# eth-cscs/conflux

Measured on NVIDIA H100. Metric: LU GFLOP/s (FP64, (2/3)N^3), higher is better.
Workload: dtype f64

## Files before the change

conflux_b200/csrc/dbg.cu:

```cuda
#include <algorithm>
#include <climits>
#include <limits>
#include <vector>

#include "../../include/conflux_b200.h"
#include "common.cuh"
#include "kernels.h"
#include "lu_state.h"

using namespace cflx;

namespace {
struct DevBuf {
    void* p = nullptr;
    ~DevBuf() { cudaFree(p); }
    int alloc(size_t bytes) {
        CFLX_CUDA(cudaMalloc(&p, bytes + 4096));
        return CFLX_OK;
    }
    template <class T>
    T* as() { return (T*)p; }
};
int check_device() {
    int n = 0;
// ... 366 lines not shown
    CFLX_TRY(dXc.alloc(sizeof(double) * (size_t)Nl * nrhs));
    CFLX_TRY(dXr.alloc(sizeof(double) * (size_t)Ml * nrhs));
    CFLX_TRY(dP.alloc(sizeof(double) * o_n));
    CFLX_TRY(dQ.alloc(sizeof(double) * o_n));
    CFLX_CUDA(cudaMemcpy(dA.p, A, sizeof(double) * a_n, cudaMemcpyHostToDevice));
    if (Xc) CFLX_CUDA(cudaMemcpy(dXc.p, Xc, sizeof(double) * (size_t)Nl * nrhs, cudaMemcpyHostToDevice));
    if (Xr) CFLX_CUDA(cudaMemcpy(dXr.p, Xr, sizeof(double) * (size_t)Ml * nrhs, cudaMemcpyHostToDevice));
    const Layout L{0, v, Kappa, Ml, Nl, Px, Py, pi, pj};
    auto run = [&]() {
        return launch_residual(m, dA.as<double>(), L, dXc.as<double>(), dXr.as<double>(), nrhs, nrhs, dP.as<double>(),
                               dQ.as<double>(), nrhs, 0);
    };
    cudaEvent_t e0, e1;
    CFLX_CUDA(cudaEventCreate(&e0));
    CFLX_CUDA(cudaEventCreate(&e1));
    if (reps < 1) reps = 1;
    CFLX_TRY(run());
    CFLX_CUDA(cudaEventRecord(e0));
    for (int r = 0; r < reps; ++r) CFLX_TRY(run());
    CFLX_CUDA(cudaEventRecord(e1));
    CFLX_CUDA(cudaEventSynchronize(e1));
    float ms = 0;
    CFLX_CUDA(cudaEventElapsedTime(&ms, e0, e1));
    if (ms_out) *ms_out = ms / reps;
    cudaEventDestroy(e0);
    cudaEventDestroy(e1);
    CFLX_CUDA(cudaMemset(dP.p, 0, sizeof(double) * o_n));
    CFLX_CUDA(cudaMemset(dQ.p, 0, sizeof(double) * o_n));
    CFLX_TRY(run());
    if (P_out) CFLX_CUDA(cudaMemcpy(P_out, dP.p, sizeof(double) * (size_t)rows * nrhs, cudaMemcpyDeviceToHost));
    if (Q_out) CFLX_CUDA(cudaMemcpy(Q_out, dQ.p, sizeof(double) * (size_t)rows * nrhs, cudaMemcpyDeviceToHost));
    CFLX_CUDA(cudaDeviceSynchronize());
    return CFLX_OK;
}

int cflx_dbg_panel(int n, int v, const double* panel, int* perm_out, double* A00_out, double* LU_out, int reps,
                   double* ms_out) {
    CFLX_TRY(check_device());
    if (n < 0 || v <= 0) return CFLX_ERR_ARG;
    const int64_t ld = std::max<int64_t>(2, round_up(n, 2));
    std::vector<double> WT((size_t)v * ld, 0.0);
    for (int r = 0; r < n; ++r)
        for (int c = 0; c < v; ++c) WT[(size_t)c * ld + r] = panel[(size_t)r * v + c];
    DevBuf dW, dW0, dA00, dA00T, dperm;
    CFLX_TRY(dW.alloc(sizeof(double) * v * ld));
    CFLX_TRY(dW0.alloc(sizeof(double) * v * ld));
    CFLX_TRY(dA00.alloc(sizeof(double) * v * v));
    CFLX_TRY(dA00T.alloc(sizeof(double) * v * v));
    CFLX_TRY(dperm.alloc(sizeof(int) * 2 * v));
    CFLX_CUDA(cudaMemcpy(dW0.p, WT.data(), sizeof(double) * v * ld, cudaMemcpyHostToDevice));
    CFLX_CUDA(cudaMemset(dA00.p, 0, sizeof(double) * v * v));
    PanelWorkspace ws{};
    CFLX_TRY(panel_workspace_create(&ws));
    cudaEvent_t e0, e1;
    CFLX_CUDA(cudaEventCreate(&e0));
    CFLX_CUDA(cudaEventCreate(&e1));
    if (reps < 1) reps = 1;
    float total = 0;
    int nb = 0, rc = CFLX_OK;
    for (int r = 0; r < reps + 1 && rc == CFLX_OK; ++r) {
        cudaMemcpyAsync(dW.p, dW0.p, sizeof(double) * v * ld, cudaMemcpyDeviceToDevice, 0);
        cudaEventRecord(e0);
        rc = launch_panel_getrf_a00(dW.as<double>(), ld, n, v, dperm.as<int>(), dA00.as<double>(), &nb, &ws, 0);
        cudaEventRecord(e1);
        if (cudaEventSynchronize(e1) != cudaSuccess) rc = CFLX_ERR_CUDA;
        float ms = 0;
        cudaEventElapsedTime(&ms, e0, e1);
        if (r > 0) total += ms;
    }
    cudaEventDestroy(e0);
    cudaEventDestroy(e1);
    if (rc == CFLX_OK && n >= v)
        rc = launch_gather_a00(dW.as<double>(), ld, dperm.as<int>(), v, nb, dA00.as<double>(), dA00T.as<double>(), 0);
    panel_workspace_destroy(&ws);
    if (rc != CFLX_OK) {
        if (rc == CFLX_ERR_CUDA) set_last_error("panel kernel failed: %s", cudaGetErrorString(cudaGetLastError()));
        return rc;
    }
    if (ms_out) *ms_out = total / reps;
    if (perm_out) CFLX_CUDA(cudaMemcpy(perm_out, dperm.p, sizeof(int) * v, cudaMemcpyDeviceToHost));
    if (A00_out) CFLX_CUDA(cudaMemcpy(A00_out, dA00.p, sizeof(double) * v * v, cudaMemcpyDeviceToHost));
    if (LU_out) {
        CFLX_CUDA(cudaMemcpy(WT.data(), dW.p, sizeof(double) * v * ld, cudaMemcpyDeviceToHost));
        for (int r = 0; r < n; ++r)
            for (int c = 0; c < v; ++c) LU_out[(size_t)r * v + c] = WT[(size_t)c * ld + r];
    }
    CFLX_CUDA(cudaDeviceSynchronize());
    return CFLX_OK;
}

int cflx_dbg_trsm(int n, int v, int nb, int64_t ld, const double* A00, const double* B, double* X_out, const double* R,
                  double* Y_out) {
    CFLX_TRY(check_device());
    if (n <= 0 || v <= 0 || v % 4 != 0) return CFLX_ERR_ARG;
    if (nb == 0)
        for (int c : {128, 64, 32, 16, 8, 4})
            if (!nb && v % c == 0) nb = c;
    if (nb != 4 && nb != 8 && nb != 16 && nb != 32 && nb != 64 && nb != 128) return CFLX_ERR_UNSUPPORTED;
    if (v % nb != 0) return CFLX_ERR_ARG;
    if (ld == 0) ld = round_up(n, 2);
    if ((ld & 1) || ld < round_up(n, 2)) return CFLX_ERR_ARG;
    const double nan = std::numeric_limits<double>::quiet_NaN();
    std::vector<double> A00T((size_t)v * v), BT((size_t)v * ld, nan), RT((size_t)v * ld, nan);
    for (int i = 0; i < v; ++i)
        for (int j = 0; j < v; ++j) A00T[(size_t)j * v + i] = A00[(size_t)i * v + j];
    DevBuf dA, dAT, dUinv, dLinvT, dP, dL, dR, dU;
// ... 191 lines not shown
```

conflux_b200/csrc/lu.cu:

```cuda
#include <algorithm>
#include <cmath>
#include <cstdarg>
#include <cstdlib>
#include <cstring>
#include <random>
#include <string>
#include <vector>

#include <nvtx3/nvToolsExt.h>

#include "lu_state.h"

namespace cflx {
static thread_local char g_err[1024] = "";
void set_last_error(const char* fmt, ...) {
    va_list ap;
    va_start(ap, fmt);
    vsnprintf(g_err, sizeof(g_err), fmt, ap);
    va_end(ap);
}
}

using namespace cflx;

// ... 811 lines not shown
    lu->a0_is_next = false;
    lu->next_host = nullptr;
    lu->eq.in.equed = 'N';
    return CFLX_OK;
}

int cflx_lu_queue_next_local(cflx_lu* lu, const double* host_next) {
    if (!lu || !host_next) return CFLX_ERR_ARG;
    if (!lu->have_input) {
        set_last_error("cflx_lu_queue_next_local needs a current input (cflx_lu_set_local) first");
        return CFLX_ERR_STATE;
    }
    CFLX_CUDA(cudaSetDevice(lu->comm->device));
    if (!lu->copy) {
        CFLX_CUDA(cudaStreamCreateWithFlags(&lu->copy, cudaStreamNonBlocking));
        CFLX_CUDA(cudaEventCreateWithFlags(&lu->ev_a0_read, cudaEventDisableTiming));
        CFLX_CUDA(cudaEventCreateWithFlags(&lu->ev_upload, cudaEventDisableTiming));
    }
    lu->next_host = host_next;
    return CFLX_OK;
}

int cflx_lu_factor(cflx_lu* lu, double* ms_out) {
    if (!lu) return CFLX_ERR_ARG;
    if (!lu->have_input) {
        set_last_error("cflx_lu_factor before cflx_lu_set_local");
        return CFLX_ERR_STATE;
    }
    cflx_comm* c = lu->comm;
    cudaStream_t s = c->stream;
    CFLX_CUDA(cudaSetDevice(c->device));
    const size_t loc = (size_t)lu->Ml * lu->Nl;
    {
        PhaseTimer t(lu, RG_init, s);
        if (lu->a0_is_next) CFLX_CUDA(cudaStreamWaitEvent(s, lu->ev_upload, 0));
        CFLX_CUDA(cudaMemcpyAsync(lu->A11, lu->A0, loc * sizeof(double), cudaMemcpyDeviceToDevice, s));
    }
    lu->a0_is_next = false;
    lu->sv.ready = false;
    CFLX_TRY(equil_pass_on(&lu->eq, lu->M, lu->next_host != nullptr, s));
    if (lu->next_host) {
        CFLX_CUDA(cudaEventRecord(lu->ev_a0_read, s));
        CFLX_CUDA(cudaStreamWaitEvent(lu->copy, lu->ev_a0_read, 0));
        CFLX_CUDA(cudaMemcpyAsync(lu->A0, lu->next_host, loc * sizeof(double), cudaMemcpyHostToDevice, lu->copy));
        CFLX_CUDA(cudaEventRecord(lu->ev_upload, lu->copy));
        lu->next_host = nullptr;
        lu->a0_is_next = true;
    }
    CFLX_TRY(launch_iota_gri(lu->gri, lu->igri, lu->Ml, lu->v, lu->Px, lu->pi, s));
    for (double& x : lu->phase_ms) x = 0;
    for (int sd = 0; sd < 2; ++sd)
        for (int r = 0; r < RG_COUNT; ++r) lu->region_ms[sd][r] = 0, lu->region_cnt[sd][r] = 0;
    lu->tl_recs.clear();
    CFLX_TRY(grid_barrier(c));
    cudaEvent_t e0, e1;
    CFLX_CUDA(cudaEventCreate(&e0));
    CFLX_CUDA(cudaEventCreate(&e1));
    CFLX_CUDA(cudaEventRecord(e0, s));
    int fnpr = 0;
    lu->gemm_flops = 0;
    lu->gemm_ms = 0;
    if (lu->time_gemm && (int)lu->ev.size() < 4 * lu->Nt) {
        for (auto& e : lu->ev) cudaEventDestroy(e);
        lu->ev.assign(4 * lu->Nt, nullptr);
        for (auto& e : lu->ev) CFLX_CUDA(cudaEventCreate(&e));
    }
    lu->ev_used.assign(2 * lu->Nt, 0);
    {
        cudaStream_t side = (lu->prof_mode == 1) ? nullptr : lu->side;
        if (side) {
            CFLX_CUDA(cudaEventRecord(lu->ev_fork, s));
            CFLX_CUDA(cudaStreamWaitEvent(side, lu->ev_fork, 0));
        }
        int rc0 = panel_phase(lu, 0, 0, side ? side : s);
        if (rc0 != CFLX_OK) return rc0;
        if (side) {
            CFLX_CUDA(cudaEventRecord(lu->ev_join, side));
            CFLX_CUDA(cudaStreamWaitEvent(s, lu->ev_join, 0));
        }
    }
    for (int k = 0; k < lu->Nt; ++k) {
        int rc = finish_step(lu, k, fnpr);
        if (rc != CFLX_OK) {
            cudaEventDestroy(e0);
            cudaEventDestroy(e1);
            return rc;
        }
    }
    CFLX_CUDA(cudaEventRecord(e1, s));
    CFLX_CUDA(cudaEventSynchronize(e1));
    float ms = 0;
    CFLX_CUDA(cudaEventElapsedTime(&ms, e0, e1));
    cudaEventDestroy(e0);
    cudaEventDestroy(e1);
    CFLX_CUDA(cudaGetLastError());
    if (ms_out) *ms_out = ms;
    if (lu->prof_mode == 2) {
        if (lu->side) cudaStreamSynchronize(lu->side);
        for (const auto& r : lu->tl_recs) {
            float g = 0;
            if (cudaEventElapsedTime(&g, lu->tl_pool[r.ev], lu->tl_pool[r.ev + 1]) == cudaSuccess) {
                lu->region_ms[r.side][r.region] += g;
                lu->region_cnt[r.side][r.region]++;
                lu->phase_ms[region_phase(r.region)] += g;
            } else {
                cudaGetLastError();
            }
        }
    }
    if (lu->time_gemm) {
        for (int i = 0; i < 2 * lu->Nt; ++i) {
            if (!lu->ev_used[i]) continue;
            float g = 0;
            if (cudaEventElapsedTime(&g, lu->ev[2 * i], lu->ev[2 * i + 1]) == cudaSuccess) lu->gemm_ms += g;
            else cudaGetLastError();
        }
    }
    if (lu->a0_is_next) CFLX_CUDA(cudaStreamSynchronize(lu->copy));
    lu->factored = true;
    return CFLX_OK;
}

int cflx_lu_get_permutation(cflx_lu* lu, int* perm_out) {
    if (!lu || !perm_out) return CFLX_ERR_ARG;
    CFLX_TRY(lu_check(lu, "permutation", false));
    CFLX_CUDA(cudaSetDevice(lu->comm->device));
    CFLX_CUDA(cudaMemcpyAsync(lu->h_hist.data(), lu->hist, sizeof(int) * lu->M, cudaMemcpyDeviceToHost, lu->comm->stream));
    CFLX_CUDA(cudaStreamSynchronize(lu->comm->stream));
    std::memcpy(perm_out, lu->h_hist.data(), sizeof(int) * lu->M);
    return CFLX_OK;
}

int cflx_lu_get_factors(cflx_lu* lu, double* C_host, int* perm_out) {
    if (!lu) return CFLX_ERR_ARG;
    CFLX_TRY(lu_check(lu, "factors", false));
    cflx_comm* c = lu->comm;
    cudaStream_t s = c->stream;
    CFLX_CUDA(cudaSetDevice(c->device));
    std::vector<int> hist(lu->M);
    CFLX_TRY(cflx_lu_get_permutation(lu, hist.data()));
    if (perm_out) std::memcpy(perm_out, hist.data(), sizeof(int) * lu->M);
    if (lu->pk != 0) return CFLX_OK;
    const size_t loc = (size_t)lu->Ml * lu->Nl;
    if (!lu->Cbuf) CFLX_TRY(dmalloc(&lu->Cbuf, loc));
    CFLX_TRY(redistribute_pivoted_rows(lu, hist, true, lu->A11, lu->Cbuf));
    if (C_host) CFLX_CUDA(cudaMemcpyAsync(C_host, lu->Cbuf, loc * sizeof(double), cudaMemcpyDeviceToHost, s));
    CFLX_CUDA(cudaStreamSynchronize(s));
    return CFLX_OK;
}

int cflx_lu_validate(cflx_lu* lu, double* frob_abs_out, double* frob_rel_out) {
    if (!lu) return CFLX_ERR_ARG;
    CFLX_TRY(lu_check(lu, "residual", true));
    CFLX_CUDA(cudaSetDevice(lu->comm->device));
    std::vector<int> hist(lu->M);
    CFLX_TRY(cflx_lu_get_permutation(lu, hist.data()));
    return lu_residual_grid(lu, hist, frob_abs_out, frob_rel_out);
// ... 98 lines not shown
    CFLX_TRY(lu_rcond(lu, t, &rcond, nullptr));
    *rcond_out = rcond;
    const double *r = rowequ ? eq.r : nullptr, *c = colequ ? eq.c : nullptr;
    const RefineOp op = lu_refine_op(lu, t);
    if (!t) CFLX_TRY(svx_tail(&lu->eq, &lu->sv.rf, op, nrhs, B, ldb, X, ldx, ferr_out, berr_out, r, c, eq.colcnd));
    else CFLX_TRY(svx_tail(&lu->eq, &lu->sv.rf, op, nrhs, B, ldb, X, ldx, ferr_out, berr_out, c, r, eq.rowcnd));
    if (rcond < std::ldexp(1.0, -53)) *info_out = lu->M + 1;
    return CFLX_OK;
}

int cflx_host_alloc(size_t bytes, void** out) {
    if (!out) return CFLX_ERR_ARG;
    int n = 0;
    cflx_device_count(&n);
    if (n == 0) {
        set_last_error("no CUDA device visible: conflux_b200 has no CPU fallback");
        return CFLX_ERR_NO_DEVICE;
    }
    CFLX_CUDA(cudaHostAlloc(out, bytes, cudaHostAllocPortable));
    return CFLX_OK;
}
int cflx_host_free(void* p) {
    if (p) CFLX_CUDA(cudaFreeHost(p));
    return CFLX_OK;
}

int cflx_lu_uses_ozaki(const cflx_lu* lu) { return lu && lu->use_ozaki ? 1 : 0; }
int cflx_lu_launch_count(cflx_lu* lu, int64_t* count_out, int reset) {
    if (!lu || !count_out) return CFLX_ERR_ARG;
    *count_out = lu->launches;
    if (reset) lu->launches = 0;
    return CFLX_OK;
}
int cflx_lu_set_profiling(cflx_lu* lu, int mode) {
    if (!lu || mode < 0 || mode > 2) return CFLX_ERR_ARG;
    lu->prof_mode = mode;
    return CFLX_OK;
}
int cflx_lu_timeline(cflx_lu* lu, char* buf, int buf_len) {
    if (!lu) return CFLX_ERR_ARG;
    std::string o = "{";
    for (int sd = 0; sd < 2; ++sd) {
        o += sd ? ", \"side\": {" : "\"main\": {";
        bool first = true;
        for (int r = 0; r < RG_COUNT; ++r) {
            if (!lu->region_cnt[sd][r]) continue;
            char tmp[160];
            snprintf(tmp, sizeof(tmp), "%s\"%s\": [%.4f, %d]", first ? "" : ", ", region_name(r), lu->region_ms[sd][r], lu->region_cnt[sd][r]);
            o += tmp;
            first = false;
        }
        o += "}";
    }
    o += "}";
    if (!buf || buf_len <= (int)o.size()) return (int)o.size() + 1;
    std::memcpy(buf, o.c_str(), o.size() + 1);
    return CFLX_OK;
}
int cflx_lu_phase_ms(cflx_lu* lu, double* ms_out) {
    if (!lu || !ms_out) return CFLX_ERR_ARG;
    for (int i = 0; i < PH_COUNT; ++i) ms_out[i] = lu->phase_ms[i];
    return CFLX_OK;
}
int cflx_lu_set_kernel_timing(cflx_lu* lu, int enabled) {
    if (!lu) return CFLX_ERR_ARG;
    lu->time_gemm = enabled != 0;
    return CFLX_OK;
}
int cflx_lu_trailing_stats(cflx_lu* lu, double* ms_out, double* flops_out) {
    if (!lu || !ms_out || !flops_out) return CFLX_ERR_ARG;
    *ms_out = lu->gemm_ms;
    *flops_out = lu->gemm_flops;
    return CFLX_OK;
}
void cflx_lu_destroy(cflx_lu* lu) { free_lu(lu); }

}
```

conflux_b200/csrc/lu_state.h:

```cpp
#pragma once
#include <nccl.h>

#include <algorithm>
#include <functional>
#include <vector>

#include "../../include/conflux_b200.h"
#include "common.cuh"
#include "kernels.h"

#define CFLX_NCCL(call)                                                                                    \
    do {                                                                                                   \
        ncclResult_t r__ = (call);                                                                         \
        if (r__ != ncclSuccess) {                                                                          \
            ::cflx::set_last_error("%s:%d: %s -> %s", __FILE__, __LINE__, #call, ncclGetErrorString(r__)); \
            return CFLX_ERR_NCCL;                                                                          \
        }                                                                                                  \
    } while (0)

struct cflx_comm {
    int world_size = 1, world_rank = 0, device = 0;
    ncclComm_t world = nullptr;
    cudaStream_t stream = nullptr;
    double* d_scratch = nullptr;
// ... 99 lines not shown
    int* rows_id = nullptr;
    int* cols = nullptr;
    int* unperm = nullptr;
    double *B = nullptr, *W = nullptr, *Z = nullptr, *R = nullptr, *Y = nullptr, *X = nullptr, *Xg = nullptr;
    int ldn = 0;
    bool col_partials = false, col_seed = false;
    RefineCache rf;
};

enum class Tri { Lower, Upper, LowerT, UnitLowerT, UpperT };

struct SolveSeed {
    bool by_col;
    const int* rows;
    int n;
    double* dst;
};

struct SolveFactor {
    const Grid& g;
    const double* F;
    int rows;
    const SubComm *row_comm, *col_comm;
    int stride;
};
}

struct cflx_lu : cflx::Grid {
    int N = 0, Mt = 0;
    cflx::SubComm jk_comm, ik_comm;
    double *A0 = nullptr, *A11 = nullptr, *PT = nullptr, *PT2 = nullptr, *W = nullptr, *LT = nullptr, *A01raw = nullptr,
           *U = nullptr, *tmp = nullptr, *A00 = nullptr, *A00T = nullptr, *Uinv = nullptr, *LinvT = nullptr,
           *candH = nullptr, *S = nullptr, *W2 = nullptr, *bcast = nullptr, *Cbuf = nullptr, *xbuf = nullptr;
    int *gri = nullptr, *gri_tmp = nullptr, *igri = nullptr, *perm = nullptr, *gpivots = nullptr, *tagsH = nullptr,
        *tagsS = nullptr, *hist = nullptr, *plan_mem = nullptr, *idx_buf = nullptr;
    cflx::MovePlan plan{};
    cflx::PanelWorkspace pws{};
    cflx::OzakiWorkspace oz{};
    bool use_ozaki = false;
    int64_t ldp_max = 0;
    int* h_npiv = nullptr;
    std::vector<int> h_hist;
    bool have_input = false, factored = false, time_gemm = false;
    const double* next_host = nullptr;
    bool a0_is_next = false;
    cudaStream_t copy = nullptr;
    cudaEvent_t ev_a0_read = nullptr, ev_upload = nullptr;
    double gemm_ms = 0, gemm_flops = 0;
    int64_t launches = 0;
    double phase_ms[cflx::PH_COUNT] = {0};
    struct TlRec { int region, side, ev; };
    std::vector<cudaEvent_t> tl_pool;
    std::vector<TlRec> tl_recs;
    double region_ms[2][cflx::RG_COUNT] = {{0}};
    int region_cnt[2][cflx::RG_COUNT] = {{0}};
    int prof_mode = 0;
    std::vector<cudaEvent_t> ev;
    std::vector<char> ev_used;
    cudaStream_t side = nullptr;
    cudaEvent_t ev_fork = nullptr, ev_join = nullptr, ev_npiv = nullptr;
    cflx::SolveCache sv;
    cflx::EquilState eq;
};

namespace cflx {
int redistribute_pivoted_rows(cflx_lu* lu, const std::vector<int>& hist, bool factors, const double* src, double* dst);
int lu_residual_grid(cflx_lu* lu, const std::vector<int>& hist, double* abs_out, double* rel_out);

void solve_cache_free(SolveCache* sc);
int solve_cache_grow(SolveCache* sc, const SolveFactor& f, int ldn, bool work, bool col_partials, bool col_seed = false);
int solve_inverses(SolveCache* sc, const SolveFactor& f, bool lower);
int solve_set_rows(int** dst, const std::vector<int>& rows, cudaStream_t s);
int solve_seed(SolveCache* sc, const SolveFactor& f, int ldn, int nrhs, const double* B, int ldb, const SolveSeed& at);
int solve_row_sweep(SolveCache* sc, const SolveFactor& f, int ldn, bool forward, double* keep, int keep_div,
                    bool clear_row, int t_lo = 0, int t_hi = -1);
int solve_col_sweep(SolveCache* sc, const SolveFactor& f, int ldn, bool forward, Tri tri, double* keep, int keep_div,
                    bool clear_col, int t_lo = 0, int t_hi = -1);
int solve_finish(SolveCache* sc, const SolveFactor& f, int ldn, int nrhs, double* X, int ldx, const int* unperm = nullptr);
int estimate_inv_norm1(int n, const std::function<int(int, double*)>& apply, double* est);
int norm1_grid(const Grid& g, const double* A, bool lower_sym, double* anorm);
double rcond_from(double anorm, double ainvnm);

struct Lacn2 {
    int n = 0, kase = 0, jump = 0, j = 0, iter = 0;
    double est = 0.0;
    bool pending = false;
    std::vector<double> x, v;
    std::vector<int> isgn;
    void start(int n);
    int step();
};

struct RefineOp {
    const Grid& grid;
    const double* A;
    ResidMode mode;
    bool symmetric;
    std::function<int(bool, int, const double*, int, double*, int)> solve;
};
int refine_run(RefineCache* rc, const RefineOp& op, int nrhs, const double* B, int ldb, double* X, int ldx, double* ferr,
               double* berr);
void refine_cache_free(RefineCache* rc);
int launch_residual(ResidMode mode, const double* A, const Layout& L, const double* Xc, const double* Xr, int64_t ldx,
                    int nrhs, double* P, double* Q, int64_t ldo, cudaStream_t s);
int svx_tail(EquilState* e, RefineCache* rc, const RefineOp& op, int nrhs, const double* B, int ldb, double* X, int ldx,
             double* ferr, double* berr, const double* pre, const double* post, double cnd);
// ... 31 lines not shown
```

conflux_b200/csrc/panel.cu:

```cuda
#include <cooperative_groups.h>

#include <climits>
#include <cstdlib>

#include "common.cuh"
#include "kernels.h"

namespace cflx {

namespace {
constexpr int PT_THREADS = 256;
constexpr int PT_WARPS = PT_THREADS / 32;
constexpr int MAXG = 132;
constexpr int RPT_LIMIT = 8;

struct PanelArgs {
    double* W;
    int64_t ldw;
    int n, v, nsteps;
    int R, Rpad, G;
    int* perm_out;
    double* A00;
    uint2* slot_hdr;
    uint2* slot_rows;
    int epoch_base;
};

__device__ __forceinline__ void st_ll(uint2* p, unsigned data, unsigned epoch) {
    asm volatile("st.volatile.global.v2.u32 [%0], {%1, %2};" ::"l"(p), "r"(data), "r"(epoch) : "memory");
}
__device__ __forceinline__ uint4 ld_ll2(const uint2* p) {
    uint4 v;
    asm volatile("ld.volatile.global.v4.u32 {%0, %1, %2, %3}, [%4];" : "=r"(v.x), "=r"(v.y), "=r"(v.z), "=r"(v.w) : "l"(p) : "memory");
    return v;
}

struct Cand {
    unsigned long long key;
    int pos;
    int row;
};

__device__ __forceinline__ Cand warp_argmax(Cand c) {
    const unsigned hi = (unsigned)(c.key >> 32), lo = (unsigned)c.key;
    const unsigned m1 = __reduce_max_sync(0xffffffffu, hi);
    bool in = (hi == m1);
    const unsigned m2 = __reduce_max_sync(0xffffffffu, in ? lo : 0u);
    in = in && (lo == m2);
    const unsigned m3 = __reduce_min_sync(0xffffffffu, in ? (unsigned)c.pos : (unsigned)INT_MAX);
    const unsigned ballot = __ballot_sync(0xffffffffu, in && (unsigned)c.pos == m3);
    const int src = __ffs(ballot) - 1;
    Cand r;
    r.key = ((unsigned long long)m1 << 32) | m2;
    r.pos = (int)m3;
    r.row = __shfl_sync(0xffffffffu, c.row, src);
    return r;
}
__device__ __forceinline__ bool better(const Cand& a, const Cand& b) {
    return a.key > b.key || (a.key == b.key && a.pos < b.pos);
}
__device__ __forceinline__ Cand block_argmax(Cand c, unsigned long long* red_key, int* red_pos, int* red_row, int& rb) {
    Cand w = warp_argmax(c);
    const int warp = threadIdx.x >> 5;
    const int o = rb * PT_WARPS;
    rb ^= 1;
    if ((threadIdx.x & 31) == 0) {
        red_key[o + warp] = w.key;
        red_pos[o + warp] = w.pos;
        red_row[o + warp] = w.row;
    }
    __syncthreads();
    Cand best{red_key[o], red_pos[o], red_row[o]};
#pragma unroll
    for (int i = 1; i < PT_WARPS; ++i) {
        Cand x{red_key[o + i], red_pos[o + i], red_row[o + i]};
        if (better(x, best)) best = x;
    }
    return best;
}

template <int NB, int RPT_MAX>
__global__ void __launch_bounds__(PT_THREADS, 1) panel_getrf_kernel(PanelArgs p) {
    extern __shared__ __align__(16) unsigned char smem_raw[];
    double* Ab = reinterpret_cast<double*>(smem_raw);
    double* U12 = Ab + (size_t)NB * p.Rpad;
    double* LU11 = U12 + (size_t)NB * p.v;
    double* prow = LU11 + NB * (NB + 1);
    unsigned long long* red_key = reinterpret_cast<unsigned long long*>(prow + 2 * NB);
    int* red_pos = reinterpret_cast<int*>(red_key + 2 * PT_WARPS);
    int* red_row = red_pos + 2 * PT_WARPS;
    int* pivrow_blk = red_row + 2 * PT_WARPS;
    int* win_sh = pivrow_blk + NB;
    unsigned char* s_act = reinterpret_cast<unsigned char*>(win_sh + 4);
    int rb = 0;

    const int t = threadIdx.x;
    const int cta = blockIdx.x;
    const int row_base = cta * p.R;
    const int Rloc = max(0, min(p.R, p.n - row_base));
    const int Rpad = p.Rpad, v = p.v;
    double* __restrict__ W = p.W;
    const int64_t ldw = p.ldw;

    int pos[RPT_MAX];
    bool active[RPT_MAX];
#pragma unroll
    for (int q = 0; q < RPT_MAX; ++q) {
        const int lr = t + q * PT_THREADS;
        pos[q] = row_base + lr;
        active[q] = lr < Rloc;
    }
    for (int lr = t; lr < Rpad; lr += PT_THREADS) s_act[lr] = lr < Rloc ? 1 : 0;

    for (int jb = 0; jb < p.nsteps; jb += NB) {
        const int nbc = min(NB, v - jb);
        const int nsb = min(nbc, p.nsteps - jb);
        for (int e = t; e < nbc * Rpad; e += PT_THREADS) {
            const int c = e / Rpad, lr = e - c * Rpad;
            if (lr < Rloc) Ab[e] = W[(int64_t)(jb + c) * ldw + row_base + lr];
        }
        __syncthreads();

        auto local_candidate = [&](int col) -> Cand {
            Cand c{0ull, INT_MAX, -1};
#pragma unroll
            for (int q = 0; q < RPT_MAX; ++q) {
                const int lr = t + q * PT_THREADS;
                if (active[q]) {
                    Cand o{(unsigned long long)__double_as_longlong(fabs(Ab[col * Rpad + lr])), pos[q], row_base + lr};
                    if (better(o, c)) c = o;
                }
            }
            return block_argmax(c, red_key, red_pos, red_row, rb);
        };
        auto publish = [&](const Cand& mine, int jg, int jprev, const double* pw) {
            const unsigned epoch = (unsigned)(p.epoch_base + jg + 1);
            const int par = jg & 1;
            uint2* myhdr = p.slot_hdr + (size_t)(par * MAXG + cta) * 4;
            if (t < 4) {
                const unsigned w = t == 0 ? (unsigned)mine.key : t == 1 ? (unsigned)(mine.key >> 32)
                                 : t == 2 ? (unsigned)mine.pos : (unsigned)mine.row;
                st_ll(myhdr + t, w, epoch);
            }
            if (t < nbc) {
                double x = 0.0;
                if (mine.row >= 0) {
                    const int lrw = mine.row - row_base;
                    x = Ab[t * Rpad + lrw];
                    if (jprev >= 0 && t > jprev + 1) x = fma(-Ab[jprev * Rpad + lrw], pw[t], x);
                }
                const unsigned long long xb = (unsigned long long)__double_as_longlong(x);
                uint2* myrow = p.slot_rows + (size_t)(par * MAXG + cta) * 64 + 2 * t;
                st_ll(myrow, (unsigned)xb, epoch);
                st_ll(myrow + 1, (unsigned)(xb >> 32), epoch);
            }
        };
        {
            const Cand mine0 = local_candidate(0);
            if (t < 32) __threadfence();
            publish(mine0, jb, -1, nullptr);
        }
        for (int j = 0; j < nsb; ++j) {
            const int jg = jb + j;
            const int par = jg & 1;
            double* pr = prow + par * NB;
            {
                const unsigned epoch = (unsigned)(p.epoch_base + jg + 1);
                Cand gc{0ull, INT_MAX, -1};
                for (int g = t; g < p.G; g += PT_THREADS) {
                    const uint2* h = p.slot_hdr + (size_t)(par * MAXG + g) * 4;
                    uint4 a, b;
                    do {
                        a = ld_ll2(h);
                        b = ld_ll2(h + 2);
                    } while (a.y != epoch || a.w != epoch || b.y != epoch || b.w != epoch);
                    Cand o{((unsigned long long)a.z << 32) | a.x, (int)b.x, (int)b.z};
                    if (better(o, gc)) gc = o;
                }
                Cand w = gc;
                if (p.G > 32) w = block_argmax(gc, red_key, red_pos, red_row, rb);
                else if (t < 32) w = warp_argmax(gc);
                if (t < nbc) {
                    const uint2* wr = p.slot_rows + (size_t)(par * MAXG + w.row / p.R) * 64 + 2 * t;
                    uint4 a;
                    do {
                        a = ld_ll2(wr);
                    } while (a.y != epoch || a.w != epoch);
                    const double x = __longlong_as_double((long long)(((unsigned long long)a.z << 32) | a.x));
                    pr[t] = x;
                    LU11[j * (NB + 1) + t] = x;
                }
                if (t == 0) {
                    win_sh[2 * par] = w.pos;
                    win_sh[2 * par + 1] = w.row;
                }
            }
            __syncthreads();
            Cand win;
            win.key = 0;
            win.pos = win_sh[2 * par];
            win.row = win_sh[2 * par + 1];
            if (t == 0) {
                pivrow_blk[j] = win.row;
                if (cta == 0) p.perm_out[jg] = win.row;
            }
            const double pivot = pr[j];
            const double rinv = pivot != 0.0 ? 1.0 / pivot : 0.0;
            const bool have_next = (j + 1 < nbc);
            const double pnext = have_next ? pr[j + 1] : 0.0;
            double lq[RPT_MAX];
#pragma unroll
            for (int q = 0; q < RPT_MAX; ++q) {
                const int lr = t + q * PT_THREADS;
                lq[q] = 0.0;
                if (!active[q]) continue;
                if (row_base + lr == win.row) {
                    active[q] = false;
                    s_act[lr] = 0;
                    continue;
                }
                if (pos[q] == jg) pos[q] = win.pos;
                if (pivot != 0.0) {
                    lq[q] = Ab[j * Rpad + lr] * rinv;
                    Ab[j * Rpad + lr] = lq[q];
                }
                if (have_next) Ab[(j + 1) * Rpad + lr] = fma(-lq[q], pnext, Ab[(j + 1) * Rpad + lr]);
            }
            if (j + 1 < nsb) {
                const Cand mine = local_candidate(j + 1);
                publish(mine, jg + 1, j, pr);
                __syncthreads();
            }
            {
                double* __restrict__ ab = Ab;
#pragma unroll 4
                for (int c2 = j + 2; c2 < nbc; ++c2) {
                    const double pc = pr[c2];
#pragma unroll
                    for (int q = 0; q < RPT_MAX; ++q) {
                        const int lr = t + q * PT_THREADS;
                        if (active[q]) ab[c2 * Rpad + lr] = fma(-lq[q], pc, ab[c2 * Rpad + lr]);
                    }
                }
            }
        }

        __syncthreads();
        for (int e = t; e < nbc * Rpad; e += PT_THREADS) {
            const int c = e / Rpad, lr = e - c * Rpad;
            if (lr < Rloc) W[(int64_t)(jb + c) * ldw + row_base + lr] = Ab[e];
        }
        if (cta == 0 && p.A00 != nullptr) {
            for (int e = t; e < nsb * nbc; e += PT_THREADS) {
                const int i = e / nbc, c = e % nbc;
                p.A00[(size_t)(jb + i) * v + jb + c] = LU11[i * (NB + 1) + c];
            }
        }

        const int cstart = jb + nbc;
        const int rem = v - cstart;
        if (rem > 0) {
            __syncthreads();
            __threadfence();
            for (int cc = t; cc < rem; cc += PT_THREADS) {
                const double* col = W + (int64_t)(cstart + cc) * ldw;
                double u[NB];
#pragma unroll
                for (int i = 0; i < NB; ++i) u[i] = (i < nsb) ? ld_cg_f64(col + pivrow_blk[i]) : 0.0;
#pragma unroll
                for (int i = 1; i < NB; ++i) {
                    if (i < nsb) {
#pragma unroll
                        for (int s2 = 0; s2 < i; ++s2) u[i] -= LU11[i * (NB + 1) + s2] * u[s2];
                    }
                }
#pragma unroll
                for (int i = 0; i < NB; ++i) U12[i * v + cc] = u[i];
                if (cta == 0 && p.A00 != nullptr) {
#pragma unroll
                    for (int i = 0; i < NB; ++i)
                        if (i < nsb) p.A00[(size_t)(jb + i) * v + cstart + cc] = u[i];
                }
            }
            __syncthreads();
            auto update_row = [&](int lr, int cfirst, int cstep, bool tail) {
                double l[NB];
#pragma unroll
                for (int i = 0; i < NB; ++i) l[i] = (i < nsb) ? Ab[i * Rpad + lr] : 0.0;
                double* wp = W + (int64_t)cstart * ldw + row_base + lr;
                int cc = cfirst;
                double w0 = 0, w1 = 0, w2 = 0, w3 = 0;
                if (cc + 3 < rem) {
                    w0 = wp[(int64_t)cc * ldw];
                    w1 = wp[(int64_t)(cc + 1) * ldw];
                    w2 = wp[(int64_t)(cc + 2) * ldw];
                    w3 = wp[(int64_t)(cc + 3) * ldw];
                }
                for (; cc + 3 < rem; cc += cstep) {
                    double n0 = 0, n1 = 0, n2 = 0, n3 = 0;
                    const int cn = cc + cstep;
                    if (cn + 3 < rem) {
                        n0 = wp[(int64_t)cn * ldw];
                        n1 = wp[(int64_t)(cn + 1) * ldw];
                        n2 = wp[(int64_t)(cn + 2) * ldw];
                        n3 = wp[(int64_t)(cn + 3) * ldw];
                    }
#pragma unroll
                    for (int i = 0; i < NB; ++i) {
                        const double2 ua = *reinterpret_cast<const double2*>(U12 + i * v + cc);
                        const double2 ub = *reinterpret_cast<const double2*>(U12 + i * v + cc + 2);
                        w0 -= l[i] * ua.x;
                        w1 -= l[i] * ua.y;
                        w2 -= l[i] * ub.x;
                        w3 -= l[i] * ub.y;
                    }
                    wp[(int64_t)cc * ldw] = w0;
                    wp[(int64_t)(cc + 1) * ldw] = w1;
                    wp[(int64_t)(cc + 2) * ldw] = w2;
                    wp[(int64_t)(cc + 3) * ldw] = w3;
                    w0 = n0;
                    w1 = n1;
                    w2 = n2;
                    w3 = n3;
                }
                if (tail) {
                    for (int ct = rem & ~3; ct < rem; ++ct) {
                        double x = wp[(int64_t)ct * ldw];
#pragma unroll
                        for (int i = 0; i < NB; ++i) x -= l[i] * U12[i * v + ct];
                        wp[(int64_t)ct * ldw] = x;
                    }
                }
            };
            if (RPT_MAX == 1 && p.R < PT_THREADS) {
                const int nshare = PT_THREADS / p.R;
                const int lr = t % p.R, part = t / p.R;
                if (part < nshare && lr < Rloc && s_act[lr]) update_row(lr, 4 * part, 4 * nshare, part == 0);
            } else {
#pragma unroll 1
                for (int q = 0; q < RPT_MAX; ++q) {
                    const int lr = t + q * PT_THREADS;
                    if (lr >= Rloc || !active[q]) continue;
                    update_row(lr, 0, 4, true);
                }
            }
        }
        __threadfence();
        __syncthreads();
    }
    if (cta == 0)
        for (int i = p.nsteps + t; i < v; i += PT_THREADS) p.perm_out[i] = i;
}

constexpr int SK_CB = 16;
struct StackArgs {
    double* W;
    int64_t ldw;
    int n, v;
    int* perm_out;
    int* ppos;
    unsigned* flags;
    unsigned* ticket;
    unsigned ticket_base, epoch;
};
__device__ __forceinline__ unsigned ld_acquire_u32(const unsigned* p) {
    unsigned v;
    asm volatile("ld.acquire.gpu.global.u32 %0, [%1];" : "=r"(v) : "l"(p) : "memory");
    return v;
}
__device__ __forceinline__ void st_release_u32(unsigned* p, unsigned v) {
    asm volatile("st.release.gpu.global.u32 [%0], %1;" ::"l"(p), "r"(v) : "memory");
}
__device__ __forceinline__ void cp_async16(double* smem_dst, const double* gsrc) {
    asm volatile("cp.async.cg.shared.global [%0], [%1], 16;" ::"r"(smem_u32(smem_dst)), "l"(gsrc) : "memory");
}
__device__ __forceinline__ void cp_async_commit() { asm volatile("cp.async.commit_group;" ::: "memory"); }
__device__ __forceinline__ void cp_async_wait_all() { asm volatile("cp.async.wait_all;" ::: "memory"); }

template <int NT>
__global__ void __launch_bounds__(NT, 1) stack_getrf_kernel(StackArgs p) {
    __shared__ double A12s[SK_CB][SK_CB + 1];
    __shared__ double L11s[SK_CB][SK_CB + 1];
    __shared__ double prow[2][SK_CB];
    __shared__ unsigned long long red_key[2][32];
    __shared__ int red_pos[2][32], red_row[2][32];
    __shared__ int pivs[SK_CB], ppos_s[SK_CB];
    __shared__ int s_cta;
    extern __shared__ __align__(16) double Ls[];
    const int t = threadIdx.x, warp = t >> 5, lane = t & 31, nw = blockDim.x >> 5;
    if (t == 0) s_cta = (int)(atomicAdd(p.ticket, 1u) - p.ticket_base);
    __syncthreads();
    const int c = s_cta, c0 = c * SK_CB;
    const bool valid = t < p.n;
    double* __restrict__ W = p.W;
    const int64_t ldw = p.ldw;
    double a[SK_CB];
#pragma unroll
    for (int j = 0; j < SK_CB; ++j) a[j] = valid ? W[(int64_t)(c0 + j) * ldw + t] : 0.0;
    int pos = t;
    int mypiv = -1;

    for (int b = 0; b < c; ++b) {
        if (t == 0)
            while (ld_acquire_u32(p.flags + b) != p.epoch) {}
// ... 78 lines not shown
        }
        __syncthreads();
        if (valid && mypiv < 0) {
            if (pos == jg) pos = win.pos;
            const double pivot = prow[par][j];
            const double rinv = pivot != 0.0 ? 1.0 / pivot : 0.0;
            double lq = 0.0;
            if (pivot != 0.0) {
                lq = a[j] * rinv;
                a[j] = lq;
            }
#pragma unroll
            for (int m = j + 1; m < SK_CB; ++m) a[m] = fma(-lq, prow[par][m], a[m]);
        }
    }
    if (valid) {
#pragma unroll
        for (int j = 0; j < SK_CB; ++j) W[(int64_t)(c0 + j) * ldw + t] = a[j];
    }
    __threadfence();
    __syncthreads();
    if (t == 0) st_release_u32(p.flags + c, p.epoch);
}

int launch_stack_getrf(double* W, int64_t ldw, int n, int v, int* perm_out, PanelWorkspace* ws, cudaStream_t stream) {
    StackArgs a{};
    a.W = W;
    a.ldw = ldw;
    a.n = n;
    a.v = v;
    a.perm_out = perm_out;
    a.ppos = ws->sk_ppos;
    a.flags = ws->sk_flags;
    a.ticket = ws->sk_ticket;
    a.ticket_base = ws->sk_ticket_count;
    a.epoch = ++ws->sk_epoch;
    const int C = v / SK_CB;
    ws->sk_ticket_count += (unsigned)C;
    const int threads = (int)round_up(n, 32);
    static PerDeviceMax cfg;
    if (cfg.raise((size_t)SK_CB * 1024 * sizeof(double))) {
        CFLX_CUDA(cudaFuncSetAttribute(stack_getrf_kernel<1024>, cudaFuncAttributeMaxDynamicSharedMemorySize, SK_CB * 1024 * 8));
        CFLX_CUDA(cudaFuncSetAttribute(stack_getrf_kernel<512>, cudaFuncAttributeMaxDynamicSharedMemorySize, SK_CB * 512 * 8));
    }
    if (threads <= 256) stack_getrf_kernel<256><<<C, threads, SK_CB * 256 * sizeof(double), stream>>>(a);
    else if (threads <= 512) stack_getrf_kernel<512><<<C, threads, SK_CB * 512 * sizeof(double), stream>>>(a);
    else stack_getrf_kernel<1024><<<C, threads, SK_CB * 1024 * sizeof(double), stream>>>(a);
    CFLX_CUDA(cudaGetLastError());
    return CFLX_OK;
}

template <int NB>
size_t panel_smem_bytes(int Rpad, int v) {
    return ((size_t)NB * Rpad + (size_t)NB * v + NB * (NB + 1) + 2 * NB) * sizeof(double) +
           2 * PT_WARPS * (sizeof(unsigned long long) + 2 * sizeof(int)) +
           (NB + 4) * sizeof(int) + (size_t)Rpad;
}

int panel_nb(int Rpad, int v) {
    for (int nb = 32; nb >= 4; nb /= 2) {
        const long long limit = 222 * 1024 - (8LL * nb * nb + 796LL * nb + 848);
        if ((nb <= v || nb == 4) && (8LL * nb + 1) * Rpad + 8LL * nb * v <= limit) return nb;
    }
    return 0;
}

template <int NB, int RPT>
int launch_nb_rpt(PanelArgs& a, cudaStream_t stream) {
    const size_t smem = panel_smem_bytes<NB>(a.Rpad, a.v);
    void* params[] = {&a};
    static PerDeviceMax cfg;
    if (cfg.raise(smem))
        CFLX_CUDA(cudaFuncSetAttribute(panel_getrf_kernel<NB, RPT>, cudaFuncAttributeMaxDynamicSharedMemorySize, (int)smem));
    CFLX_CUDA(cudaLaunchCooperativeKernel((void*)panel_getrf_kernel<NB, RPT>, dim3(a.G), dim3(PT_THREADS), params, smem, stream));
    return CFLX_OK;
}
template <int NB>
int launch_nb(PanelArgs& a, cudaStream_t stream) {
    const int rpt = (a.R + PT_THREADS - 1) / PT_THREADS;
    if (rpt <= 1) return launch_nb_rpt<NB, 1>(a, stream);
    if (rpt <= 2) return launch_nb_rpt<NB, 2>(a, stream);
    if (rpt <= 4) return launch_nb_rpt<NB, 4>(a, stream);
    return launch_nb_rpt<NB, 8>(a, stream);
}
}

int panel_workspace_create(PanelWorkspace* ws) {
    int dev = 0, sms = 0;
    CFLX_CUDA(cudaGetDevice(&dev));
    CFLX_CUDA(cudaDeviceGetAttribute(&sms, cudaDevAttrMultiProcessorCount, dev));
    ws->max_ctas = sms < MAXG ? sms : MAXG;
    ws->epoch = 1;
    ws->cta_cap = 0;
    CFLX_CUDA(cudaMalloc(&ws->slot_hdr, sizeof(uint2) * 2 * MAXG * 4));
    CFLX_CUDA(cudaMalloc(&ws->slot_rows, sizeof(uint2) * 2 * MAXG * 64));
    CFLX_CUDA(cudaMemset(ws->slot_hdr, 0, sizeof(uint2) * 2 * MAXG * 4));
    CFLX_CUDA(cudaMemset(ws->slot_rows, 0, sizeof(uint2) * 2 * MAXG * 64));
    CFLX_CUDA(cudaMalloc(&ws->sk_flags, sizeof(unsigned) * 1024));
    CFLX_CUDA(cudaMalloc(&ws->sk_ppos, sizeof(int) * 16384));
    CFLX_CUDA(cudaMalloc(&ws->sk_ticket, sizeof(unsigned)));
    CFLX_CUDA(cudaMemset(ws->sk_flags, 0, sizeof(unsigned) * 1024));
    CFLX_CUDA(cudaMemset(ws->sk_ticket, 0, sizeof(unsigned)));
    ws->sk_epoch = 0;
    ws->sk_ticket_count = 0;
    {
        const char* e = getenv("CFLX_STACK_KERNEL");
        ws->sk_enabled = e ? atoi(e) : 1;
    }
    return CFLX_OK;
}
void panel_workspace_destroy(PanelWorkspace* ws) {
    cudaFree(ws->slot_hdr);
    cudaFree(ws->slot_rows);
    cudaFree(ws->sk_flags);
    cudaFree(ws->sk_ppos);
    cudaFree(ws->sk_ticket);
    *ws = PanelWorkspace{};
}

int launch_panel_getrf_a00(double* W, int64_t ldw, int n, int v, int* perm_out, double* A00, int* nb_used,
                           PanelWorkspace* ws, cudaStream_t stream) {
    if (v <= 0 || n < 0) return CFLX_ERR_ARG;
    if (ws->sk_enabled && n >= v && n <= 1024 && v % SK_CB == 0 && v <= 16384 && ldw % 2 == 0 &&
        (reinterpret_cast<uintptr_t>(W) & 15) == 0) {
        if (nb_used) *nb_used = 0;
        return launch_stack_getrf(W, ldw, n, v, perm_out, ws, stream);
    }
    PanelArgs a{};
    a.W = W;
    a.ldw = ldw;
    a.n = n;
    a.v = v;
    a.nsteps = n < v ? n : v;
    int G = (n + 31) / 32;
    if (G < 1) G = 1;
    if (G > ws->max_ctas) G = ws->max_ctas;
    if (ws->cta_cap > 0 && G > ws->cta_cap) {
        G = ws->cta_cap;
// ... 41 lines not shown
```

Before: 23920.

## Add dedicated fetcher warp for pivot exchange in panel getrf kernel

Launches the panel LU kernel with an extra warp. When the grid has at most 32 CTAs, that warp alone polls the other CTAs' pivot slots and fetches the winning row, while the 256 owner threads do the row updates. The winning slot is now found with a ballot, and the pivot reciprocal is computed once and stored in shared memory. The block-wide argmax now finishes with a warp shuffle reduction instead of a serial loop. This adds a warp of register and shared-memory pressure and changes the synchronisation structure. It also adds timeline span recording and a Python model of the exchange protocol.

New measurement: 25280 (median of 6 runs). 5.7% higher.

```diff
diff --git a/conflux_b200/csrc/dbg.cu b/conflux_b200/csrc/dbg.cu
--- a/conflux_b200/csrc/dbg.cu
+++ b/conflux_b200/csrc/dbg.cu
@@ -442,6 +442,7 @@
     CFLX_CUDA(cudaMemset(dA00.p, 0, sizeof(double) * v * v));
     PanelWorkspace ws{};
     CFLX_TRY(panel_workspace_create(&ws));
+    if (const char* e = getenv("CFLX_PANEL_CTAS")) ws.cta_cap = atoi(e);
     cudaEvent_t e0, e1;
     CFLX_CUDA(cudaEventCreate(&e0));
     CFLX_CUDA(cudaEventCreate(&e1));
diff --git a/conflux_b200/csrc/lu.cu b/conflux_b200/csrc/lu.cu
--- a/conflux_b200/csrc/lu.cu
+++ b/conflux_b200/csrc/lu.cu
@@ -887,6 +887,7 @@
     for (int sd = 0; sd < 2; ++sd)
         for (int r = 0; r < RG_COUNT; ++r) lu->region_ms[sd][r] = 0, lu->region_cnt[sd][r] = 0;
     lu->tl_recs.clear();
+    lu->tl_spans.clear();
     CFLX_TRY(grid_barrier(c));
     cudaEvent_t e0, e1;
     CFLX_CUDA(cudaEventCreate(&e0));
@@ -938,6 +939,9 @@
                 lu->region_ms[r.side][r.region] += g;
                 lu->region_cnt[r.side][r.region]++;
                 lu->phase_ms[region_phase(r.region)] += g;
+                float st = 0;
+                if (cudaEventElapsedTime(&st, lu->tl_pool[0], lu->tl_pool[r.ev]) != cudaSuccess) cudaGetLastError();
+                lu->tl_spans.push_back({r.region, r.side, st, g});
             } else {
                 cudaGetLastError();
             }
@@ -1142,7 +1146,15 @@
         }
         o += "}";
     }
-    o += "}";
+    o += ", \"records\": [";
+    for (size_t i = 0; i < lu->tl_spans.size(); ++i) {
+        const auto& sp = lu->tl_spans[i];
+        char tmp[160];
+        snprintf(tmp, sizeof(tmp), "%s[\"%s\", \"%s\", %.4f, %.4f]", i ? ", " : "", region_name(sp.region), sp.side ? "side" : "main",
+                 sp.start_ms, sp.ms);
+        o += tmp;
+    }
+    o += "]}";
     if (!buf || buf_len <= (int)o.size()) return (int)o.size() + 1;
     std::memcpy(buf, o.c_str(), o.size() + 1);
     return CFLX_OK;
diff --git a/conflux_b200/csrc/lu_state.h b/conflux_b200/csrc/lu_state.h
--- a/conflux_b200/csrc/lu_state.h
+++ b/conflux_b200/csrc/lu_state.h
@@ -175,6 +175,8 @@
     struct TlRec { int region, side, ev; };
     std::vector<cudaEvent_t> tl_pool;
     std::vector<TlRec> tl_recs;
+    struct TlSpan { int region, side; float start_ms, ms; };
+    std::vector<TlSpan> tl_spans;
     double region_ms[2][cflx::RG_COUNT] = {{0}};
     int region_cnt[2][cflx::RG_COUNT] = {{0}};
     int prof_mode = 0;
diff --git a/conflux_b200/csrc/panel.cu b/conflux_b200/csrc/panel.cu
--- a/conflux_b200/csrc/panel.cu
+++ b/conflux_b200/csrc/panel.cu
@@ -11,6 +11,8 @@
 namespace {
 constexpr int PT_THREADS = 256;
 constexpr int PT_WARPS = PT_THREADS / 32;
+constexpr int PT_LAUNCH = PT_THREADS + 32;
+constexpr int PT_ALLWARPS = PT_LAUNCH / 32;
 constexpr int MAXG = 132;
 constexpr int RPT_LIMIT = 8;
 
@@ -61,40 +63,39 @@
 }
 __device__ __forceinline__ Cand block_argmax(Cand c, unsigned long long* red_key, int* red_pos, int* red_row, int& rb) {
     Cand w = warp_argmax(c);
-    const int warp = threadIdx.x >> 5;
-    const int o = rb * PT_WARPS;
+    const int warp = threadIdx.x >> 5, lane = threadIdx.x & 31;
+    const int o = rb * PT_ALLWARPS;
     rb ^= 1;
-    if ((threadIdx.x & 31) == 0) {
+    if (lane == 0) {
         red_key[o + warp] = w.key;
         red_pos[o + warp] = w.pos;
         red_row[o + warp] = w.row;
     }
     __syncthreads();
-    Cand best{red_key[o], red_pos[o], red_row[o]};
-#pragma unroll
-    for (int i = 1; i < PT_WARPS; ++i) {
-        Cand x{red_key[o + i], red_pos[o + i], red_row[o + i]};
-        if (better(x, best)) best = x;
-    }
-    return best;
+    Cand x{0ull, INT_MAX, -1};
+    if (lane < PT_ALLWARPS) x = Cand{red_key[o + lane], red_pos[o + lane], red_row[o + lane]};
+    return warp_argmax(x);
 }
 
 template <int NB, int RPT_MAX>
-__global__ void __launch_bounds__(PT_THREADS, 1) panel_getrf_kernel(PanelArgs p) {
+__global__ void __launch_bounds__(PT_LAUNCH, 1) panel_getrf_kernel(PanelArgs p) {
     extern __shared__ __align__(16) unsigned char smem_raw[];
     double* Ab = reinterpret_cast<double*>(smem_raw);
     double* U12 = Ab + (size_t)NB * p.Rpad;
     double* LU11 = U12 + (size_t)NB * p.v;
     double* prow = LU11 + NB * (NB + 1);
-    unsigned long long* red_key = reinterpret_cast<unsigned long long*>(prow + 2 * NB);
-    int* red_pos = reinterpret_cast<int*>(red_key + 2 * PT_WARPS);
-    int* red_row = red_pos + 2 * PT_WARPS;
-    int* pivrow_blk = red_row + 2 * PT_WARPS;
+    unsigned long long* red_key = reinterpret_cast<unsigned long long*>(prow + 2 * (NB + 1));
+    int* red_pos = reinterpret_cast<int*>(red_key + 2 * PT_ALLWARPS);
+    int* red_row = red_pos + 2 * PT_ALLWARPS;
+    int* pivrow_blk = red_row + 2 * PT_ALLWARPS;
     int* win_sh = pivrow_blk + NB;
     unsigned char* s_act = reinterpret_cast<unsigned char*>(win_sh + 4);
     int rb = 0;
 
-    const int t = threadIdx.x;
+    const int t = threadIdx.x, warp = t >> 5, lane = t & 31;
+    const bool owner = t < PT_THREADS;
+    const bool small = p.G <= 32;
+    const bool fetcher = warp == (small ? PT_WARPS : 0);
     const int cta = blockIdx.x;
     const int row_base = cta * p.R;
     const int Rloc = max(0, min(p.R, p.n - row_base));
@@ -108,14 +109,14 @@
     for (int q = 0; q < RPT_MAX; ++q) {
         const int lr = t + q * PT_THREADS;
         pos[q] = row_base + lr;
-        active[q] = lr < Rloc;
-    }
-    for (int lr = t; lr < Rpad; lr += PT_THREADS) s_act[lr] = lr < Rloc ? 1 : 0;
+        active[q] = owner && lr < Rloc;
+    }
+    for (int lr = t; lr < Rpad; lr += PT_LAUNCH) s_act[lr] = lr < Rloc ? 1 : 0;
 
     for (int jb = 0; jb < p.nsteps; jb += NB) {
         const int nbc = min(NB, v - jb);
         const int nsb = min(nbc, p.nsteps - jb);
-        for (int e = t; e < nbc * Rpad; e += PT_THREADS) {
+        for (int e = t; e < nbc * Rpad; e += PT_LAUNCH) {
             const int c = e / Rpad, lr = e - c * Rpad;
             if (lr < Rloc) Ab[e] = W[(int64_t)(jb + c) * ldw + row_base + lr];
         }
@@ -163,11 +164,11 @@
         for (int j = 0; j < nsb; ++j) {
             const int jg = jb + j;
             const int par = jg & 1;
-            double* pr = prow + par * NB;
-            {
+            double* pr = prow + par * (NB + 1);
+            if (!small || fetcher) {
                 const unsigned epoch = (unsigned)(p.epoch_base + jg + 1);
                 Cand gc{0ull, INT_MAX, -1};
-                for (int g = t; g < p.G; g += PT_THREADS) {
+                for (int g = small ? lane : t; g < p.G; g += small ? 32 : PT_LAUNCH) {
                     const uint2* h = p.slot_hdr + (size_t)(par * MAXG + g) * 4;
                     uint4 a, b;
                     do {
@@ -177,20 +178,20 @@
                     Cand o{((unsigned long long)a.z << 32) | a.x, (int)b.x, (int)b.z};
                     if (better(o, gc)) gc = o;
                 }
-                Cand w = gc;
-                if (p.G > 32) w = block_argmax(gc, red_key, red_pos, red_row, rb);
-                else if (t < 32) w = warp_argmax(gc);
-                if (t < nbc) {
-                    const uint2* wr = p.slot_rows + (size_t)(par * MAXG + w.row / p.R) * 64 + 2 * t;
+                const Cand w = small ? warp_argmax(gc) : block_argmax(gc, red_key, red_pos, red_row, rb);
+                const int wslot = small ? __ffs(__ballot_sync(0xffffffffu, gc.row == w.row)) - 1 : w.row / p.R;
+                if (fetcher && lane < nbc) {
+                    const uint2* wr = p.slot_rows + (size_t)(par * MAXG + wslot) * 64 + 2 * lane;
                     uint4 a;
                     do {
                         a = ld_ll2(wr);
                     } while (a.y != epoch || a.w != epoch);
                     const double x = __longlong_as_double((long long)(((unsigned long long)a.z << 32) | a.x));
-                    pr[t] = x;
-                    LU11[j * (NB + 1) + t] = x;
-                }
-                if (t == 0) {
+                    pr[lane] = x;
+                    LU11[j * (NB + 1) + lane] = x;
+                    if (lane == j) pr[NB] = x != 0.0 ? 1.0 / x : 0.0;
+                }
+                if (fetcher && lane == 0) {
                     win_sh[2 * par] = w.pos;
                     win_sh[2 * par + 1] = w.row;
                 }
@@ -205,7 +206,7 @@
                 if (cta == 0) p.perm_out[jg] = win.row;
             }
             const double pivot = pr[j];
-            const double rinv = pivot != 0.0 ? 1.0 / pivot : 0.0;
+            const double rinv = pr[NB];
             const bool have_next = (j + 1 < nbc);
             const double pnext = have_next ? pr[j + 1] : 0.0;
             double lq[RPT_MAX];
@@ -231,7 +232,7 @@
                 publish(mine, jg + 1, j, pr);
                 __syncthreads();
             }
-            {
+            if (owner) {
                 double* __restrict__ ab = Ab;
 #pragma unroll 4
                 for (int c2 = j + 2; c2 < nbc; ++c2) {
@@ -246,12 +247,12 @@
         }
 
         __syncthreads();
-        for (int e = t; e < nbc * Rpad; e += PT_THREADS) {
+        for (int e = t; e < nbc * Rpad; e += PT_LAUNCH) {
             const int c = e / Rpad, lr = e - c * Rpad;
             if (lr < Rloc) W[(int64_t)(jb + c) * ldw + row_base + lr] = Ab[e];
         }
         if (cta == 0 && p.A00 != nullptr) {
-            for (int e = t; e < nsb * nbc; e += PT_THREADS) {
+            for (int e = t; e < nsb * nbc; e += PT_LAUNCH) {
                 const int i = e / nbc, c = e % nbc;
                 p.A00[(size_t)(jb + i) * v + jb + c] = LU11[i * (NB + 1) + c];
             }
@@ -262,7 +263,7 @@
         if (rem > 0) {
             __syncthreads();
             __threadfence();
-            for (int cc = t; cc < rem; cc += PT_THREADS) {
+            for (int cc = t; cc < rem; cc += PT_LAUNCH) {
                 const double* col = W + (int64_t)(cstart + cc) * ldw;
                 double u[NB];
 #pragma unroll
@@ -335,7 +336,7 @@
             if (RPT_MAX == 1 && p.R < PT_THREADS) {
                 const int nshare = PT_THREADS / p.R;
                 const int lr = t % p.R, part = t / p.R;
-                if (part < nshare && lr < Rloc && s_act[lr]) update_row(lr, 4 * part, 4 * nshare, part == 0);
+                if (owner && part < nshare && lr < Rloc && s_act[lr]) update_row(lr, 4 * part, 4 * nshare, part == 0);
             } else {
 #pragma unroll 1
                 for (int q = 0; q < RPT_MAX; ++q) {
@@ -349,7 +350,7 @@
         __syncthreads();
     }
     if (cta == 0)
-        for (int i = p.nsteps + t; i < v; i += PT_THREADS) p.perm_out[i] = i;
+        for (int i = p.nsteps + t; i < v; i += PT_LAUNCH) p.perm_out[i] = i;
 }
 
 constexpr int SK_CB = 16;
@@ -534,8 +535,8 @@
 
 template <int NB>
 size_t panel_smem_bytes(int Rpad, int v) {
-    return ((size_t)NB * Rpad + (size_t)NB * v + NB * (NB + 1) + 2 * NB) * sizeof(double) +
-           2 * PT_WARPS * (sizeof(unsigned long long) + 2 * sizeof(int)) +
+    return ((size_t)NB * Rpad + (size_t)NB * v + NB * (NB + 1) + 2 * (NB + 1)) * sizeof(double) +
+           2 * PT_ALLWARPS * (sizeof(unsigned long long) + 2 * sizeof(int)) +
            (NB + 4) * sizeof(int) + (size_t)Rpad;
 }
 
@@ -554,7 +555,7 @@
     static PerDeviceMax cfg;
     if (cfg.raise(smem))
         CFLX_CUDA(cudaFuncSetAttribute(panel_getrf_kernel<NB, RPT>, cudaFuncAttributeMaxDynamicSharedMemorySize, (int)smem));
-    CFLX_CUDA(cudaLaunchCooperativeKernel((void*)panel_getrf_kernel<NB, RPT>, dim3(a.G), dim3(PT_THREADS), params, smem, stream));
+    CFLX_CUDA(cudaLaunchCooperativeKernel((void*)panel_getrf_kernel<NB, RPT>, dim3(a.G), dim3(PT_LAUNCH), params, smem, stream));
     return CFLX_OK;
 }
 template <int NB>
@@ -566,6 +567,7 @@
     return launch_nb_rpt<NB, 8>(a, stream);
 }
 }
+
 
 int panel_workspace_create(PanelWorkspace* ws) {
     int dev = 0, sms = 0;
diff --git a/oracle/panel_exchange_ref.py b/oracle/panel_exchange_ref.py
--- /dev/null
+++ b/oracle/panel_exchange_ref.py
@@ -0,0 +1,151 @@
+import random
+
+
+class ExchangeError(AssertionError):
+    pass
+
+
+HDR = 4
+
+
+def candidate(launch, g, j, nrow):
+    h = (launch * 7919 + g * 104729 + j * 1299709) & 0xFFFFFFFF
+    h = (h * 2654435761) & 0xFFFFFFFF
+    key = h % 5
+    pos = (h >> 8) % 1000 * 64 + g
+    row = g * 1000 + j
+    return (key, pos, row), tuple((row, c) for c in range(nrow))
+
+
+def better(a, b):
+    return a[0] > b[0] or (a[0] == b[0] and a[1] < b[1])
+
+
+class Model:
+    def __init__(self, G, ncols, nrow=3, early_publish=False):
+        assert 1 <= G <= 32
+        self.G, self.ncols, self.nrow, self.early = G, ncols, nrow, early_publish
+        self.slots = [[[(None, 0, None)] * (HDR + nrow) for _ in range(G)] for _ in range(2)]
+        self.epoch_base = 0
+        self.launch = 0
+
+    def run(self, rng):
+        G, ncols = self.G, self.ncols
+        self.gather_done = [-1] * G
+        self.seen = [[None] * ncols for _ in range(G)]
+        self.bar = [dict() for _ in range(G)]
+        agents = []
+        for g in range(G):
+            agents.append(self._owners(g))
+            agents.append(self._gather(g))
+        waiting = [None] * len(agents)
+        live = set(range(len(agents)))
+        while live:
+            ready = [i for i in sorted(live) if self._ready(waiting[i])]
+            if not ready:
+                raise ExchangeError("(ii) no progress: a gather can never complete")
+            i = rng.choice(ready)
+            try:
+                waiting[i] = next(agents[i])
+            except StopIteration:
+                live.discard(i)
+        for j in range(ncols):
+            first = self.seen[0][j]
+            for g in range(1, G):
+                if self.seen[g][j] != first:
+                    raise ExchangeError(f"(iii) column {j}: CTA 0 saw {first}, CTA {g} saw {self.seen[g][j]}")
+        out = [self.seen[0][j] for j in range(ncols)]
+        self.epoch_base += ncols + 2 + (ncols & 1)
+        self.launch += 1
+        return out
+
+    def _ready(self, st):
+        if st is None:
+            return True
+        if st[0] == "bar":
+            return self.bar[st[1]].get(st[2], 0) >= 2
+        _, par, g, words, epoch = st
+        return all(self.slots[par][g][w][1] == epoch for w in words)
+
+    def _barrier(self, g, name):
+        self.bar[g][name] = self.bar[g].get(name, 0) + 1
+        return ("bar", g, name)
+
+    def _publish(self, g, j):
+        epoch = self.epoch_base + j + 1
+        par = j & 1
+        cand, row = candidate(self.launch, g, j, self.nrow)
+        words = [cand[0], 0, cand[1], cand[2]] + list(row)
+        for w, payload in enumerate(words):
+            old = self.slots[par][g][w]
+            if old[2] is not None and old[2][0] == self.launch:
+                oldcol = old[2][1]
+                late = [c for c in range(self.G) if self.gather_done[c] < oldcol]
+                if late:
+                    raise ExchangeError(f"(i) CTA {g} overwrites word {w} of column {oldcol} with column {j} before "
+                                        f"CTAs {late} finished that gather")
+            self.slots[par][g][w] = (payload, epoch, (self.launch, j))
+            yield None
+
+    def _owners(self, g):
+        published = -1
+        for j in range(self.ncols):
+            yield self._barrier(g, ("B1", j))
+            if published < j:
+                yield from self._publish(g, j)
+                published = j
+            if j > 0:
+                yield self._barrier(g, ("B2", j))
+            yield None
+            if self.early and j + 1 < self.ncols:
+                yield from self._publish(g, j + 1)
+                published = j + 1
+            yield self._barrier(g, ("R", j))
+
+    def _gather(self, g):
+        for j in range(self.ncols):
+            yield self._barrier(g, ("B1", j))
+            if j > 0:
+                yield self._barrier(g, ("B2", j))
+            epoch = self.epoch_base + j + 1
+            par = j & 1
+            best, slot = None, -1
+            for s in range(self.G):
+                while True:
+                    ws = []
+                    for w in range(HDR):
+                        ws.append(self.slots[par][s][w])
+                    if all(x[1] == epoch for x in ws):
+                        break
+                    yield ("spin", par, s, tuple(range(HDR)), epoch)
+                cand = (ws[0][0], ws[2][0], ws[3][0])
+                if best is None or better(cand, best):
+                    best, slot = cand, s
+                yield None
+            row = []
+            for w in range(HDR, HDR + self.nrow):
+                while self.slots[par][slot][w][1] != epoch:
+                    yield ("spin", par, slot, (w,), epoch)
+                row.append(self.slots[par][slot][w][0])
+                yield None
+            self.seen[g][j] = (best, tuple(row))
+            self.gather_done[g] = j
+            yield self._barrier(g, ("R", j))
+
+
+def run(G, ncols, seed, launches=1, early_publish=False, nrow=3):
+    rng = random.Random(seed)
+    m = Model(G, ncols, nrow=nrow, early_publish=early_publish)
+    return [m.run(rng) for _ in range(launches)]
+
+
+def expected(G, ncols, launch=0, nrow=3):
+    out = []
+    for j in range(ncols):
+        best = None
+        for g in range(G):
+            cand, row = candidate(launch, g, j, nrow)
+            if best is None or better(cand, best[0]):
+                best = (cand, row)
+        out.append(best)
+    return out
```
